# jcatalang/LUDVM

Hardware: AMD Instinct MI355X
Metric: biot_savart_pair_interactions_per_s (higher is better)
Workload: dtype f32

## Files before the change

ludvm_amd/csrc/context.hip:

```cpp
#include "ctx.hpp"

namespace ludvm_host {

int fail(ludvm_ctx* c, int code, const std::string& msg) {
  if (c) c->err = msg;
  return code;
}

int fail_hip(ludvm_ctx* c, const char* what, hipError_t e) {
  return fail(c, e == hipErrorOutOfMemory ? LUDVM_E_NOMEM : LUDVM_E_HIP,
              std::string(what) + ": " + hipGetErrorString(e));
}

int ensure(ludvm_ctx* c, Buf& b, size_t bytes) {
  if (bytes <= b.cap) return LUDVM_OK;
  HIPCHK(c, hipStreamSynchronize(c->stream));
  if (c->stream_b) HIPCHK(c, hipStreamSynchronize(c->stream_b));
  if (b.p) HIPCHK(c, hipFree(b.p));
  b.p = nullptr;
  b.cap = 0;
  size_t want = std::max(bytes, (size_t)1 << 20);
  HIPCHK(c, hipMalloc(&b.p, want));
  b.cap = want;
  return LUDVM_OK;
}

int h2d(ludvm_ctx* c, void* dst, const void* src, size_t bytes) {
  if (bytes == 0) return LUDVM_OK;
  if (bytes > kPinBytes / 4) {
    HIPCHK(c, hipMemcpyAsync(dst, src, bytes, hipMemcpyHostToDevice, c->stream));
    HIPCHK(c, hipStreamSynchronize(c->stream));
    return LUDVM_OK;
  }
  if (!c->pin) HIPCHK(c, hipHostMalloc(reinterpret_cast<void**>(&c->pin), kPinBytes, hipHostMallocDefault));
  const size_t need = (bytes + 63) & ~(size_t)63;
  if (c->pin_off + need > kPinBytes) {
    HIPCHK(c, hipStreamSynchronize(c->stream));
    c->pin_off = 0;
  }
  std::memcpy(c->pin + c->pin_off, src, bytes);
  HIPCHK(c, hipMemcpyAsync(dst, c->pin + c->pin_off, bytes, hipMemcpyHostToDevice, c->stream));
  c->pin_off += need;
  return LUDVM_OK;
}

int d2h_small_sync(ludvm_ctx* c, const void* dsrc, size_t bytes, void** host_view) {
  if (!c->pin_out) HIPCHK(c, hipHostMalloc(reinterpret_cast<void**>(&c->pin_out), kPinOutBytes, hipHostMallocDefault));
  HIPCHK(c, hipMemcpyAsync(c->pin_out, dsrc, bytes, hipMemcpyDeviceToHost, c->stream));
  HIPCHK(c, hipStreamSynchronize(c->stream));
  *host_view = c->pin_out;
  return LUDVM_OK;
}

}

extern "C" {

int ludvm_abi_version(void) { return LUDVM_ABI_VERSION; }

int ludvm_create(int device_ordinal, ludvm_ctx** out) {
  const char* small_env = LUDVM_EXP_ENV("LUDVM_SMALL_TILE_MAX");
  if (!out) return LUDVM_E_ARG;
  *out = nullptr;
  int ndev = 0;
  if (hipGetDeviceCount(&ndev) != hipSuccess || ndev <= 0) return LUDVM_E_NODEVICE;
  if (device_ordinal < 0 || device_ordinal >= ndev) return LUDVM_E_ARG;
  ludvm_ctx* c = new (std::nothrow) ludvm_ctx();
  if (!c) return LUDVM_E_NOMEM;
  c->device = device_ordinal;
  if (hipSetDevice(device_ordinal) != hipSuccess || hipGetDeviceProperties(&c->prop, device_ordinal) != hipSuccess) {
    delete c;
    return LUDVM_E_HIP;
  }
  if (std::strncmp(c->prop.gcnArchName, "gfx950", 6) != 0) {
    delete c;
    return LUDVM_E_NODEVICE;
  }
  if (hipStreamCreateWithFlags(&c->own_stream, hipStreamNonBlocking) != hipSuccess) {
    delete c;
    return LUDVM_E_HIP;
  }
  c->stream = c->own_stream;
  if (const char* gk = LUDVM_EXP_ENV("LUDVM_GRID_KERNEL")) {
    const std::string k(gk);
    c->grid_kernel = k == "row" || k == "1" ? 1 : (k == "patch2" ? 3 : (k == "patch4" ? 4 : 2));
  }
  if (const char* fp = LUDVM_EXP_ENV("LUDVM_FEW_PACKED")) c->few_packed = !(fp[0] == '0');
  if (const char* sq = LUDVM_EXP_ENV("LUDVM_SYM_QUAD")) c->sym_quad = !(sq[0] == '0');
  if (const char* sq = LUDVM_EXP_ENV("LUDVM_SYM_QUAD_MIN_TILES")) c->sym_quad_min_tiles = std::max<long long>(16, std::atoll(sq));
  if (const char* xr = LUDVM_EXP_ENV("LUDVM_XCD_RUN")) c->xcd_run = std::max(0, std::atoi(xr));
  if (const char* ti = LUDVM_EXP_ENV("LUDVM_SYM_TAIL_ITEMS")) c->sym_tail_items = std::max<long long>(0, std::atoll(ti));
  if (const char* mx = LUDVM_EXP_ENV("LUDVM_SYM_MIXED")) {
    if (mx[0] == '1') c->tune_sym_rsplit = -1;
    if (mx[0] == '0') c->tune_sym_rsplit = -2;
  }
  if (small_env) { c->small_tile_max = std::atoll(small_env); c->small_tile_max_f64 = std::min<long long>(c->small_tile_max, 12000); }
  const char* small64_env = LUDVM_EXP_ENV("LUDVM_SMALL_TILE_MAX_F64");
  if (small64_env) c->small_tile_max_f64 = std::atoll(small64_env);
  *out = c;
  return LUDVM_OK;
}

int ludvm_destroy(ludvm_ctx* c) {
  if (!c) return LUDVM_E_ARG;
  (void)hipSetDevice(c->device);
  (void)hipStreamSynchronize(c->stream);
  if (c->stream_b) (void)hipStreamSynchronize(c->stream_b);
  comm_release(c);
  for (auto& t : c->pending) { (void)hipEventDestroy(t.e0); (void)hipEventDestroy(t.e1); }
  for (auto& t : c->pool) { (void)hipEventDestroy(t.e0); (void)hipEventDestroy(t.e1); }
  void* bufs[] = {c->part.p, c->acc.p, c->symsc.p, c->arena.p, c->orderws.p, c->x64, c->z64, c->g64, c->xh, c->xl, c->zh, c->zl, c->g32,
                  c->xr, c->zr, c->cx, c->cz, c->march_tab.p, c->march_kin.p, c->march_rows.p, c->march_state.p, c->march_hist.p,
                  c->probe_xz.p, c->probe_shift.p, c->probe_part.p, c->probe_out.p, c->tracer_seed.p, c->tracer_release.p,
                  c->tracer_shift.p, c->tracer_cur.p, c->tracer_part.p, c->tracer_out.p, c->survey_xz.p, c->survey_shift.p, c->survey_sums.p,
                  c->survey_part.p, c->ens_in.p, c->ens_work.p, c->ens_out.p};
  for (void* p : bufs)
    if (p) (void)hipFree(p);
  for (auto& e : c->march_ev)
    if (e) (void)hipEventDestroy(e);
  if (c->ev_fork) (void)hipEventDestroy(c->ev_fork);
  if (c->ev_join) (void)hipEventDestroy(c->ev_join);
  if (c->stream_b) (void)hipStreamDestroy(c->stream_b);
  if (c->progress) (void)hipHostFree(c->progress);
  if (c->pin) (void)hipHostFree(c->pin);
  if (c->pin_out) (void)hipHostFree(c->pin_out);
  if (c->own_stream) (void)hipStreamDestroy(c->own_stream);
  delete c;
  return LUDVM_OK;
}

const char* ludvm_last_error(const ludvm_ctx* c) { return c ? c->err.c_str() : "null context"; }

int ludvm_device_info(ludvm_ctx* c, int* cu_count, int* clock_khz, long long* hbm_bytes, char* name, int name_len) {
  if (!c) return LUDVM_E_ARG;
  if (cu_count) *cu_count = c->prop.multiProcessorCount;
  if (clock_khz) *clock_khz = c->prop.clockRate;
  if (hbm_bytes) *hbm_bytes = (long long)c->prop.totalGlobalMem;
  if (name && name_len > 0) {
    std::snprintf(name, (size_t)name_len, "%s (%s)", c->prop.name, c->prop.gcnArchName);
  }
  return LUDVM_OK;
}

int ludvm_set_stream(ludvm_ctx* c, void* hip_stream, int external) {
  if (!c) return LUDVM_E_ARG;
  HIPCHK(c, hipSetDevice(c->device));
  hipStream_t next = external ? static_cast<hipStream_t>(hip_stream) : c->own_stream;
  if (next == c->stream) return LUDVM_OK;
  HIPCHK(c, hipStreamSynchronize(c->stream));
  c->pin_off = 0;
  c->stream = next;
  return LUDVM_OK;
}

int ludvm_synchronize(ludvm_ctx* c) {
  if (!c) return LUDVM_E_ARG;
  HIPCHK(c, hipSetDevice(c->device));
  HIPCHK(c, hipStreamSynchronize(c->stream));
  return LUDVM_OK;
}

int ludvm_set_tuning(ludvm_ctx* c, int targets_per_lane, int source_splits) {
  if (!c) return LUDVM_E_ARG;
  if (!(targets_per_lane == 0 || targets_per_lane == 1 || targets_per_lane == 2 || targets_per_lane == 4))
    return fail(c, LUDVM_E_ARG, "targets_per_lane must be 0, 1, 2 or 4");
  if (source_splits < 0 || source_splits > kMaxSplit) return fail(c, LUDVM_E_ARG, "source_splits out of range");
  c->tune_tpl = targets_per_lane;
  c->tune_split = source_splits;
  return LUDVM_OK;
}

int ludvm_set_sym_tuning(ludvm_ctx* c, int vortices_per_lane, int rotation_split) {
// ... 42 lines not shown
```

ludvm_amd/csrc/ctx.hpp:

```cpp
#pragma once
#pragma GCC visibility push(default)
#include "../../include/ludvm_hip.h"
#pragma GCC visibility pop
#include "pair_kernels.hpp"
#include "pair_sym_kernels.hpp"
#include "march_types.hpp"
#include "spatial_order.hpp"

#include <hip/hip_ext.h>
#include <rccl/rccl.h>
#include <dlfcn.h>

#include <algorithm>
#include <cmath>
#include <cstdio>
#include <cstdlib>
#include <cstring>
#include <string>
#include <utility>
#include <vector>

using namespace ludvm;

#ifdef LUDVM_EXPERIMENTS
#define LUDVM_EXP_ENV(name) std::getenv(name)
#else
#define LUDVM_EXP_ENV(name) static_cast<const char*>(nullptr)
#endif

struct Buf {
  void* p = nullptr;
  size_t cap = 0;
};

struct TimedLaunch {
  hipEvent_t e0, e1;
};

struct ludvm_ctx {
  int device = 0;
  hipStream_t own_stream = nullptr;
  hipStream_t stream = nullptr;
  hipDeviceProp_t prop;
  std::string err;

  int tune_tpl = 0;
  int tune_split = 0;
  int sym_mode = 1;
  int tune_sym_t = 0, tune_sym_rsplit = 0;
  int xcd_run = 0;
  long long sym_tail_items = kSymTailItems;
  int grid_kernel = 2;
  long long small_tile_max = 14000;
  bool sym_quad = true;
  long long sym_quad_min_tiles = kSymQuadMinTiles;
  bool few_packed = true;
  long long small_tile_max_f64 = 12000;

  Buf part;
  Buf acc;
  Buf symsc;
  Buf arena;
  Buf orderws;
  char* pin = nullptr;
  size_t pin_off = 0;
  char* pin_out = nullptr;
  std::vector<double> pack;

  size_t wake_cap = 0, wake_n = 0;
  double *x64 = nullptr, *z64 = nullptr, *g64 = nullptr;
  float *xh = nullptr, *xl = nullptr, *zh = nullptr, *zl = nullptr, *g32 = nullptr;
  float *xr = nullptr, *zr = nullptr, *cx = nullptr, *cz = nullptr;
  Mirrors mir() const { return Mirrors{xh, xl, zh, zl, xr, zr, cx, cz}; }

  Buf march_tab, march_kin, march_rows, march_state, march_hist;
  MarchSetup msetup{};
  size_t march_kin_rows = 0;
  double march_vcore = 0.0;
  bool march_ready = false;
  unsigned long long* progress = nullptr;
  unsigned long long* progress_dev = nullptr;
  hipEvent_t march_ev[2] = {nullptr, nullptr};
  hipStream_t stream_b = nullptr;
  hipEvent_t ev_fork = nullptr, ev_join = nullptr;
  Buf probe_xz, probe_shift, probe_part, probe_out;
  size_t probe_count = 0;
  size_t probe_rows = 0;
  bool probe_shifted = false;
  Buf tracer_seed, tracer_release, tracer_shift, tracer_cur, tracer_part, tracer_out;
  size_t tracer_count = 0;
  bool tracer_shifted = false;
  bool tracer_ran = false;
  std::vector<long long> tracer_record;
  std::vector<long long> tracer_rows;
  Buf survey_xz, survey_shift, survey_sums, survey_part;
  size_t survey_count = 0;
  bool survey_shifted = false;
  long long survey_first = 1, survey_stop = 0, survey_every = 1;
  long long survey_samples = 0;

  Buf ens_in, ens_work, ens_out;

  int shard_rank = 0, shard_world = 1;
  long long shard_min_n = 0;
  ludvm_allreduce_fn reduce_hook = nullptr;
  void* reduce_user = nullptr;
  void* ext_acc = nullptr;
  size_t ext_acc_bytes = 0;
  ncclComm_t comm = nullptr;
  int comm_rank = 0, comm_world = 1;
  bool comm_force = false;

  bool timing = false;
  std::vector<TimedLaunch> pending;
  std::vector<TimedLaunch> pool;
  double total_ms = 0.0;
  long long launches = 0;
};

namespace ludvm_host {

int fail(ludvm_ctx* c, int code, const std::string& msg);
int fail_hip(ludvm_ctx* c, const char* what, hipError_t e);

#define HIPCHK(c, call)                                     \
  do {                                                      \
    hipError_t e__ = (call);                                \
    if (e__ != hipSuccess) return fail_hip((c), #call, e__); \
  } while (0)

#define CHK(call)                     \
  do {                                \
    int rc__ = (call);                \
    if (rc__ != LUDVM_OK) return rc__; \
  } while (0)

int ensure(ludvm_ctx* c, Buf& b, size_t bytes);
constexpr size_t kPinBytes = (size_t)1 << 20;
// ... 108 lines not shown
```

ludvm_amd/csrc/launch.hip:

```cpp
#include "ctx.hpp"
#include "sym_prepare_kernels.hpp"

namespace ludvm_host {

Plan make_plan(const ludvm_ctx* c, long long nt_launch, long long ns, int precision, bool small_ok, long long plan_nt, bool grid_patch) {
  Plan p{};
  const long long nt = plan_nt > 0 ? plan_nt : nt_launch;
  const bool f64 = precision == LUDVM_PREC_F64;
  p.tile = f64 ? ((nt <= kFewTargets || ns <= c->small_tile_max_f64) ? kTileF64Few : kTileF64) : kTileF32;
  if (!f64 && small_ok && ns <= c->small_tile_max) p.tile = kTileF32Small;
  if (f64) {
    p.tpl = 1;
  } else if (c->tune_tpl == 1 || c->tune_tpl == 2 || c->tune_tpl == 4) {
    p.tpl = c->tune_tpl;
  } else {
    p.tpl = nt >= 131072 ? 2 : 1;
  }
  if (p.tile == kTileF32Small && (p.tpl != 1 || nt > 65536)) p.tile = kTileF32;
  const long long per_wg = grid_patch ? (long long)kBlock * 4 * (nt >= (1LL << 20) ? 4 : 2) : (long long)kBlock * p.tpl;
  const long long ttiles = std::max<long long>(1, (nt + per_wg - 1) / per_wg);
  const long long max_split = std::max<long long>(1, (ns + p.tile - 1) / p.tile);
  long long nsplit = c->tune_split > 0 ? c->tune_split : (kTargetBlocks + ttiles - 1) / ttiles;
  nsplit = std::max<long long>(1, std::min<long long>(std::min<long long>(nsplit, max_split), kMaxSplit));
  long long chunk = (std::max<long long>(ns, 1) + nsplit - 1) / nsplit;
// ... 101 lines not shown
        else hipLaunchKernelGGL((pair_f32<4, kTileF32, false, 1, true>), grid, dim3(kBlock), 0, c->stream, a);
      }
    } else if (p.tile == kTileF32Small) {
      hipLaunchKernelGGL((pair_f32<1, kTileF32Small, false, 0, true>), grid, dim3(kBlock), 0, c->stream, a);
    } else {
      switch (p.tpl) {
        case 1: hipLaunchKernelGGL((pair_f32<1, kTileF32, false, 0, true>), grid, dim3(kBlock), 0, c->stream, a); break;
        case 2: hipLaunchKernelGGL((pair_f32<2, kTileF32, false, 0, true>), grid, dim3(kBlock), 0, c->stream, a); break;
        default: hipLaunchKernelGGL((pair_f32<4, kTileF32, false, 0, true>), grid, dim3(kBlock), 0, c->stream, a); break;
      }
    }
  } else if (p.tile == kTileF32Small && !(a.grid_nz > 0)) {
    if (precision == LUDVM_PREC_F32X2)
      hipLaunchKernelGGL((pair_f32<1, kTileF32Small, true>), grid, dim3(kBlock), 0, c->stream, a);
    else
      hipLaunchKernelGGL((pair_f32<1, kTileF32Small, false>), grid, dim3(kBlock), 0, c->stream, a);
  } else if (precision == LUDVM_PREC_F32X2) {
    switch (p.tpl) {
      case 1: hipLaunchKernelGGL((pair_f32<1, kTileF32, true>), grid, dim3(kBlock), 0, c->stream, a); break;
      case 2: hipLaunchKernelGGL((pair_f32<2, kTileF32, true>), grid, dim3(kBlock), 0, c->stream, a); break;
      default: hipLaunchKernelGGL((pair_f32<4, kTileF32, true>), grid, dim3(kBlock), 0, c->stream, a); break;
    }
  } else if (a.grid_nz > 0 && a.grid_nz % 4 == 0 && c->tune_tpl == 0) {
    const int prows = grid_patch_rows(c, a, p);
    grid = dim3((unsigned)grid_kernel_blocks(a, prows), grid.y, 1);
    if (prows == 4) {
      hipLaunchKernelGGL((pair_f32<16, kTileF32, false, 2>), grid, dim3(kBlock), 0, c->stream, a);
    } else if (prows == 2) {
      if (p.tile == kTileF32Small) hipLaunchKernelGGL((pair_f32<8, kTileF32Small, false, 2>), grid, dim3(kBlock), 0, c->stream, a);
      else hipLaunchKernelGGL((pair_f32<8, kTileF32, false, 2>), grid, dim3(kBlock), 0, c->stream, a);
    } else {
      if (p.tile == kTileF32Small) hipLaunchKernelGGL((pair_f32<4, kTileF32Small, false, 1>), grid, dim3(kBlock), 0, c->stream, a);
      else hipLaunchKernelGGL((pair_f32<4, kTileF32, false, 1>), grid, dim3(kBlock), 0, c->stream, a);
    }
  } else {
    switch (p.tpl) {
      case 1: hipLaunchKernelGGL((pair_f32<1, kTileF32, false>), grid, dim3(kBlock), 0, c->stream, a); break;
      case 2: hipLaunchKernelGGL((pair_f32<2, kTileF32, false>), grid, dim3(kBlock), 0, c->stream, a); break;
      default: hipLaunchKernelGGL((pair_f32<4, kTileF32, false>), grid, dim3(kBlock), 0, c->stream, a); break;
    }
  }
  HIPCHK(c, hipGetLastError());
  CHK(timed_end(c, t, active));
  return LUDVM_OK;
}

int induce_device(ludvm_ctx* c, const PairArgs& a, long long nt, long long ns, int precision, void* u, void* w,
                  long long plan_nt) {
  if (nt == 0) return LUDVM_OK;
  const size_t elt = precision == LUDVM_PREC_F64 ? sizeof(double) : sizeof(float);
  if (ns == 0) {
    HIPCHK(c, hipMemsetAsync(u, 0, (size_t)nt * elt, c->stream));
    HIPCHK(c, hipMemsetAsync(w, 0, (size_t)nt * elt, c->stream));
    return LUDVM_OK;
  }
  const bool grid_generic = a.grid_nz > 0 && !(a.grid_nz % 4 == 0 && c->tune_tpl == 0);
  const bool grid_patch = a.grid_nz > 0 && !grid_generic && precision == LUDVM_PREC_F32;
  Plan p = make_plan(c, nt, ns, precision, !grid_generic, plan_nt, grid_patch);
  CHK(launch_pair(c, a, p, precision, u, w));
  if (p.nsplit > 1) {
    if (precision == LUDVM_PREC_F64)
      hipLaunchKernelGGL(finish_sum<double>, dim3(blocks_for(nt)), dim3(kBlock), 0, c->stream,
                         static_cast<const double*>(c->part.p), nt, p.nt_pad, p.nsplit, static_cast<double*>(u),
                         static_cast<double*>(w));
    else
      hipLaunchKernelGGL(finish_sum<float>, dim3(blocks_for(nt)), dim3(kBlock), 0, c->stream,
                         static_cast<const float*>(c->part.p), nt, p.nt_pad, p.nsplit, static_cast<float*>(u),
                         static_cast<float*>(w));
    HIPCHK(c, hipGetLastError());
  }
  return LUDVM_OK;
}

static_assert(64 * 8 == LUDVM_SYM_TILE, "the multi-GPU entry points always use the 512-vortex tile");

SymKnobs sym_knobs(const ludvm_ctx* c) {
  SymKnobs k;
  k.sym_mode = c->sym_mode;
  k.tile_t = c->tune_sym_t;
  k.tune_split = c->tune_split;
  k.tune_rsplit = c->tune_sym_rsplit;
  k.quad = c->sym_quad;
  k.quad_min_tiles = c->sym_quad_min_tiles;
  k.tail_items = c->sym_tail_items;
  return k;
}
long long sym_threshold(const ludvm_ctx* c, bool march) { return sym_min_n(sym_knobs(c), march); }
bool use_symmetric(const ludvm_ctx* c, long long n, double vc4, bool march) {
  return sym_use(sym_knobs(c), n, (float)vc4 > 0.0f, march);
}
int sym_tile_t(const ludvm_ctx* c, long long n, bool hilo) { return sym_tile(sym_knobs(c), n, hilo); }

int launch_sym_tiles(ludvm_ctx* c, int T, const SymOperands& o, long long n, long long i_first, long long i_count, double vc4,
                     const long long* n_dev, long long n_lo, bool sharded) {
  if (n >= (1LL << 31)) return fail(c, LUDVM_E_ARG, "the symmetric kernel indexes vortices with 32 bits: n < 2^31");
  SymArgs a{};
  a.x = o.x; a.z = o.z; a.g = o.g; a.n = n;
  a.n_dev = n_dev;
  a.xl = o.xl; a.zl = o.zl;
  a.cx = o.cx; a.cz = o.cz;
  const SymKnobs k = sym_knobs(c);
  const SymVariant v = sym_variant(k, n, T, o.xl && o.zl);
  const SymGeom& gm = v.g;
  a.tune_split = k.tune_split;
  a.tune_rsplit = v.tune_rsplit;
  a.shard_rank = (n_dev && sharded) ? c->shard_rank : 0;
  a.shard_world = (n_dev && sharded) ? c->shard_world : 1;
  a.tail_items = k.tail_items;
  a.ntiles = gm.ntiles;
  a.dmax = gm.dmax;
  a.i_first = i_first;
  a.i_count = i_count;
  a.ysplit = gm.ysplit;
  a.rsplit = gm.rsplit;
  a.ytail = gm.ytail;
  a.rbulk = gm.rbulk;
  a.xcd_run = c->xcd_run;
  a.acc_u = o.acc_u;
  a.acc_w = o.acc_w;
  a.scale = o.scale;
  a.bad = o.bad;
  a.vc4 = (float)vc4;
  long long blocks = sym_blocks(i_count, gm.ysplit, gm.rsplit, gm.ytail, gm.rbulk, c->xcd_run);
  if (n_dev) blocks = std::max(blocks, sym_grid_bound(k, v, false, n_lo, n, c->xcd_run));
  if (!n_dev && i_count == 0) return LUDVM_OK;
  blocks = std::max<long long>(blocks, 1);
  if (v.quad) {
    if (i_first % 4 != 0 || (i_count % 4 != 0 && i_first + i_count != gm.ntiles))
      return fail(c, LUDVM_E_ARG, "symmetric kernel, quad variant: an owner's tile block must start and end on multiples of 4 tiles");
    TimedLaunch tq{};
    bool act = false;
    CHK(timed_begin(c, tq, act));
    SymArgs d = a;
    d.diag_only = 1;
    const long long dblocks = std::max<long long>(1, sym_blocks(n_dev ? gm.ntiles : i_count, 1, 1, 0, 1, c->xcd_run));
    hipLaunchKernelGGL((pair_sym_f32<8, false, 1>), dim3((unsigned)dblocks), dim3(kBlock), 0, c->stream, d);
    long long qblocks = quad_blocks(n_dev ? gm.ntiles : i_count, v.q.ysplit, c->xcd_run);
    if (n_dev) qblocks = std::max(qblocks, sym_grid_bound(k, v, true, n_lo, n, c->xcd_run));
    hipLaunchKernelGGL((pair_sym_quad_f32<8>), dim3((unsigned)std::max<long long>(qblocks, 1)), dim3(kBlock), 0, c->stream, a);
    HIPCHK(c, hipGetLastError());
    CHK(timed_end(c, tq, act));
    return LUDVM_OK;
  }
  TimedLaunch t{};
  bool active = false;
  CHK(timed_begin(c, t, active));
  const dim3 grid((unsigned)blocks);
  const dim3 blk(kBlock);
#define LUDVM_SYM_LAUNCH(TT, HH)                                                                              \
  switch (gm.rsplit) {                                                                                        \
    case 0: hipLaunchKernelGGL((pair_sym_f32<TT, HH, 0>), grid, blk, 0, c->stream, a); break;                 \
    case 1: hipLaunchKernelGGL((pair_sym_f32<TT, HH, 1>), grid, blk, 0, c->stream, a); break;                 \
    case 2: hipLaunchKernelGGL((pair_sym_f32<TT, HH, 2>), grid, blk, 0, c->stream, a); break;                 \
    default: hipLaunchKernelGGL((pair_sym_f32<TT, HH, 4>), grid, blk, 0, c->stream, a); break;                \
  }
  if (v.hilo) { LUDVM_SYM_LAUNCH(4, true) }
  else if (v.T == 8) { LUDVM_SYM_LAUNCH(8, false) }
  else { LUDVM_SYM_LAUNCH(4, false) }
#undef LUDVM_SYM_LAUNCH
  HIPCHK(c, hipGetLastError());
  CHK(timed_end(c, t, active));
  return LUDVM_OK;
}

int acc_buffer(ludvm_ctx* c, long long nt_pad, long long** acc) {
  const size_t bytes = ((size_t)2 * (size_t)nt_pad + 2) * sizeof(long long);
  if (c->ext_acc) {
    if (bytes > c->ext_acc_bytes) return fail(c, LUDVM_E_NOMEM, "the accumulator buffer given to ludvm_set_shard is too small");
    *acc = static_cast<long long*>(c->ext_acc) + 2;
    return LUDVM_OK;
  }
  CHK(ensure(c, c->acc, bytes));
  *acc = static_cast<long long*>(c->acc.p) + 2;
  return LUDVM_OK;
}

bool sharded_at(const ludvm_ctx* c, long long n) { return (c->shard_world > 1 || c->comm_force) && n >= c->shard_min_n; }

void shard_tiles(const ludvm_ctx* c, long long ntiles, long long* first, long long* count) {
  unsigned long long f, cnt;
  shard_block((unsigned long long)ntiles, c->shard_rank, c->shard_world, &f, &cnt);
  *first = (long long)f;
  *count = (long long)cnt;
}

int launch_sym_prepare(ludvm_ctx* c, const float* g, long long n, double vc4, SymScale* scale, long long* bad) {
  const long long nparts = (n + kPrepChunk - 1) / kPrepChunk;
  if (nparts <= 1) {
    hipLaunchKernelGGL(sym_prepare, dim3(1), dim3(kPrepBlock), 0, c->stream, g, n, vc4, scale, bad, (double*)nullptr);
  } else {
    CHK(ensure(c, c->symsc, 128 + (size_t)nparts * sizeof(double)));
    double* partial = reinterpret_cast<double*>(static_cast<char*>(c->symsc.p) + 128);
    hipLaunchKernelGGL(sym_prepare, dim3((unsigned)nparts), dim3(kPrepBlock), 0, c->stream, g, n, vc4, scale, bad, partial);
    hipLaunchKernelGGL(sym_prepare_final, dim3(1), dim3(64), 0, c->stream, partial, (int)nparts, vc4, scale, bad);
  }
  HIPCHK(c, hipGetLastError());
  return LUDVM_OK;
}

int launch_sym(ludvm_ctx* c, SymOperands o, long long n, double vc4, long long* nt_pad_out, const long long** acc_out,
               const long long** bad_out, const long long* n_dev, long long n_lo) {
  const long long nt_pad = (n + 63) / 64 * 64;
  long long* acc = nullptr;
  CHK(acc_buffer(c, nt_pad, &acc));
  CHK(ensure(c, c->symsc, 128 + (size_t)((n + kPrepChunk - 1) / kPrepChunk) * sizeof(double)));
  HIPCHK(c, hipMemsetAsync(acc - 2, 0, ((size_t)2 * (size_t)nt_pad + 2) * sizeof(long long), c->stream));
  o.acc_u = acc;
  o.acc_w = acc + nt_pad;
  if (!o.scale) {
    CHK(launch_sym_prepare(c, o.g, n, vc4, ctx_scale(c), ctx_bad(c)));
    o.scale = ctx_scale(c);
    o.bad = ctx_bad(c);
  }
  const bool sharded = sharded_at(c, n);
  if (sharded) o.bad = acc - 2;
  const int T = sym_tile_t(c, n, o.xl && o.zl);
  const long long ntiles = (n + 64LL * T - 1) / (64LL * T);
  long long first = 0, count = ntiles;
  if (sharded) shard_tiles(c, ntiles, &first, &count);
  CHK(launch_sym_tiles(c, T, o, n, first, count, vc4, n_dev, n_lo, sharded));
  if (sharded) CHK(reduce_accumulators(c, acc, nt_pad));
  *nt_pad_out = nt_pad;
// ... 50 lines not shown
```

ludvm_amd/csrc/pair_sym_kernels.hpp:

```cpp
#pragma once
#include <hip/hip_runtime.h>
#include "pair_kernels.hpp"
#include "sym_rule.hpp"

namespace ludvm {

struct SymScale {
  float scale;
  float pad;
  double inv;
};

struct SymArgs {
  const float* x; const float* z; const float* g;
  const float* xl; const float* zl;
  const float* cx; const float* cz;
  long long n;
  long long ntiles;
  long long dmax;
  long long i_first;
  long long i_count;
  int ysplit;
  int rsplit;
  int ytail;
// ... 520 lines not shown
      const int d = D - w;
      const unsigned Iw = I0 + (unsigned)w;
      const bool own = Iw < i_first + i_count && Iw < ntiles;
      return own && ((d >= 1 && d <= (int)dmax) || (even && d == dtot && Iw < ntiles / 2));
    };
    const bool valid = valid_of(wv);
    const bool any = valid_of(0) || valid_of(1) || valid_of(2) || valid_of(3);
    if (any) store_quarter();
    Org oj[NS];
#pragma unroll
    for (int q = 0; q < NS; ++q) oj[q] = to_scalars(poj[q]);
    __syncthreads();
    if (dd + 1 < per) fetch_quarter(dd + 1);
    if (!any) continue;
    f32x2 bu[H], bw[H];
#pragma unroll
    for (int m = 0; m < H; ++m) { bu[m] = (f32x2){0.f, 0.f}; bw[m] = (f32x2){0.f, 0.f}; }
    if (valid) {
#pragma unroll
      for (int q = 0; q < NS; ++q) {
        if (local) refer_targets(oj[q]);
        for (int k = 0; k < 64; k += 2) {
          const int pos0 = ((k & 32) ? lane32x4 : lane * 4) + (k & 31) * 4;
#pragma unroll
          for (int rr = 0; rr < 2; ++rr) {
            const int pos = pos0 + 4 * rr;
            f32x2 xj[2], zj[2], gj[2];
            load_plane(lx, q, pos, xj); load_plane(lz, q, pos, zj); load_plane(lg, q, pos, gj);
#pragma unroll
            for (int mm = 0; mm < 2; ++mm) {
              const int m = 2 * q + mm;
#pragma unroll
              for (int t = 0; t < T; ++t) {
                const f32x2 dx = pk_sub_sel(xq[rr][t / 2], xj[mm], t & 1);
                const f32x2 dz = pk_sub_sel(zq[rr][t / 2], zj[mm], t & 1);
                f32x2 r2 = dx * dx;
                r2 = __builtin_elementwise_fma(dz, dz, r2);
                const f32x2 qq = __builtin_elementwise_fma(r2, r2, vc4);
                const f32x2 sv = {__builtin_amdgcn_rsqf(qq.x), __builtin_amdgcn_rsqf(qq.y)};
                const f32x2 sj = sv * gj[mm];
                const f32x2 si = pk_mul_sel(sv, gp[t / 2], t & 1, sj);
                au[t] = __builtin_elementwise_fma(dz, sj, au[t]);
                aw[t] = __builtin_elementwise_fma(dx, sj, aw[t]);
                bu[m] = __builtin_elementwise_fma(dz, si, bu[m]);
                bw[m] = __builtin_elementwise_fma(dx, si, bw[m]);
              }
            }
#pragma unroll
            for (int mm = 0; mm < 2; ++mm) { bu[2 * q + mm] = dpp_rol1(bu[2 * q + mm]); bw[2 * q + mm] = dpp_rol1(bw[2 * q + mm]); }
          }
        }
      }
    }
#pragma unroll
    for (int m = 0; m < H; ++m) {
      ex[wv][(4 * m + 0) * 64 + lane] = bu[m].x; ex[wv][(4 * m + 1) * 64 + lane] = bu[m].y;
      ex[wv][(4 * m + 2) * 64 + lane] = bw[m].x; ex[wv][(4 * m + 3) * 64 + lane] = bw[m].y;
    }
    __syncthreads();
#pragma unroll 1
    for (int c = wv; c < 2 * T; c += kWaves) {
      float v = 0.0f;
#pragma unroll
      for (int w = 0; w < kWaves; ++w) v += ex[w][c * 64 + lane];
      const unsigned j = J * W + lane + 64u * (2 * (c / 4) + (c & 1));
      if (j < n) fx_add((c & 2) ? &a.acc_w[j] : &a.acc_u[j], -v, fxs);
    }
  }

  if (mine) {
#pragma unroll
    for (int t = 0; t < T; ++t) {
      const unsigned i = I * W + lane + 64u * t;
      if (i < n) {
        const float su = au[t].x + au[t].y, sw = aw[t].x + aw[t].y;
        fx_add(&a.acc_u[i], su, fxs); fx_add(&a.acc_w[i], sw, fxs);
        chk += su + sw;
      }
    }
  }
  if (!(__builtin_fabsf(chk) < __builtin_inff())) atomicAdd(reinterpret_cast<unsigned long long*>(a.bad), 1ULL);
}

constexpr int kPrepBlock = 1024;
__device__ __forceinline__ void sym_scale_from_sum(double sum_abs, double vc4, SymScale* out, long long* bad) {
  const double vc = sqrt(sqrt(vc4));
  const double bound = sum_abs / (1.4142135623730951 * vc);
  int e = 0;
  if (bound > 0.0 && bound < 1.0e300) (void)frexp(bound, &e);
  else if (!(bound == 0.0) && bad) atomicAdd(reinterpret_cast<unsigned long long*>(bad), 1ULL);
  int k = 61 - e;
  if (k > 120) k = 120;
  if (k < -120) k = -120;
  out->scale = (float)ldexp(1.0, k);
  out->pad = 0.0f;
  out->inv = ldexp(1.0, -k);
}

__device__ __forceinline__ double block_abs_sum(const float* g, long long first, long long count) {
  __shared__ double part[kPrepBlock / 64];
  double s[8] = {0, 0, 0, 0, 0, 0, 0, 0};
  const long long end = first + count;
  long long i = first + threadIdx.x;
  for (; i + 7 * kPrepBlock < end; i += 8 * kPrepBlock) {
#pragma unroll
    for (int k = 0; k < 8; ++k) s[k] += (double)__builtin_fabsf(g[i + k * kPrepBlock]);
  }
  for (int k = 0; i < end; i += kPrepBlock, ++k) s[k & 7] += (double)__builtin_fabsf(g[i]);
  double t = ((s[0] + s[1]) + (s[2] + s[3])) + ((s[4] + s[5]) + (s[6] + s[7]));
#pragma unroll
  for (int off = 32; off > 0; off >>= 1) t += __shfl_down(t, off, 64);
  __syncthreads();
  if ((threadIdx.x & 63) == 0) part[threadIdx.x >> 6] = t;
  __syncthreads();
  double tot = 0.0;
  for (int w = 0; w < (int)(blockDim.x >> 6); ++w) tot += part[w];
  return tot;
}

constexpr long long kPrepChunk = 65536;

__device__ __forceinline__ float fx_read(const long long* acc, long long i, const SymScale* sc, bool bad) {
  if (bad) return __builtin_nanf("");
  return (float)((double)acc[i] * sc->inv);
}
__device__ __forceinline__ float fx_read(const long long* acc, long long i, const SymScale* sc, const long long* bad) {
  return fx_read(acc, i, sc, *bad != 0);
}

constexpr int kFoilChunk = 256;
__device__ __forceinline__ void staged_sources_on(bool on, double xi, double zi, const double* x64, const double* z64,
                                                  const float* g32, long long first, int nsrc, float vc4, float& fu,
                                                  float& fw, int nextra = 0, const double* extra = nullptr) {
  __shared__ float fx[kFoilChunk], fz[kFoilChunk], fg[kFoilChunk];
  fu = 0.0f; fw = 0.0f;
  const int ntot = nsrc + nextra;
  if (ntot <= 0) return;
  const double ax = nsrc > 0 ? x64[first] : extra[0], az = nsrc > 0 ? z64[first] : extra[2];
  const float xr = (float)(xi - ax), zr = (float)(zi - az);
  for (int base = 0; base < ntot; base += kFoilChunk) {
    const int cnt = ntot - base < kFoilChunk ? ntot - base : kFoilChunk;
    __syncthreads();
    for (int t = threadIdx.x; t < cnt; t += blockDim.x) {
      const int q = base + t;
      if (q < nsrc) {
        fx[t] = (float)(x64[first + q] - ax);
        fz[t] = (float)(z64[first + q] - az);
        fg[t] = g32[first + q];
      } else {
        fx[t] = (float)(extra[q - nsrc] - ax);
        fz[t] = (float)(extra[2 + q - nsrc] - az);
        fg[t] = (float)extra[4 + q - nsrc];
      }
    }
    __syncthreads();
    if (on) {
      for (int j = 0; j < cnt; ++j) {
        const float dx = xr - fx[j], dz = zr - fz[j];
        const float r2 = __builtin_fmaf(dz, dz, dx * dx);
        const float k = fg[j] * __builtin_amdgcn_rsqf(__builtin_fmaf(r2, r2, vc4));
        fu = __builtin_fmaf(dz, k, fu);
        fw = __builtin_fmaf(dx, k, fw);
      }
    }
  }
}
// ... 3 lines not shown
```

ludvm_amd/csrc/sym_rule.hpp:

```cpp
#pragma once
#include <cstddef>
#include <cstdio>
#ifndef __HIPCC__
#define __host__
#define __device__
#endif

namespace ludvm {

constexpr long long kSymTargetWaves = 8 * 65536;
constexpr long long kSymMaxSplit = 64;
constexpr long long kSymMaxSplitTuned = 1024;
constexpr long long kXcds = 8;
constexpr long long kSymMaxRsplit = 4;
constexpr long long kSymMinItems = 10500;
constexpr long long kSymTailItems = 1536;
struct SymGeom { long long ntiles, dmax, dtot; int ysplit, rsplit, ytail, rbulk; };
struct XcdShare { unsigned lo, n; };
__host__ __device__ inline XcdShare xcd_share(unsigned units, unsigned e) {
  const unsigned lo = (unsigned)((unsigned long long)units * e / (unsigned)kXcds);
  return XcdShare{lo, (unsigned)((unsigned long long)units * (e + 1) / (unsigned)kXcds) - lo};
}
__host__ __device__ inline unsigned xcd_run(unsigned ys, int k) {
  return k > 0 ? (unsigned)k : (ys > 0 ? (ys + (unsigned)kXcds - 1) / (unsigned)kXcds : 1);
// ... 95 lines not shown
    rbulk = (int)rb;
  } else {
    while (rs < (I)kSymMaxRsplit && nt1 * ys * rs < (I)kSymMinItems) rs *= 2;
    if (tune_rsplit != -2 && rs < (I)kSymMaxRsplit) {
      rbulk = (int)rs;
      rs = 0;
      const I yt = (tail_items + nt1 - 1) / nt1;
      ytail = (int)(yt > ys ? ys : yt);
    }
  }
  ysplit = (int)ys;
  rsplit = (int)rs;
}
__host__ __device__ inline SymGeom sym_geometry(long long n, int T, int tune_split, int tune_rsplit,
                                                 long long tail_items = kSymTailItems) {
  SymGeom g;
  sym_geometry_t<long long>(n, T, tune_split, tune_rsplit, tail_items, g.ntiles, g.dmax, g.dtot, g.ysplit, g.rsplit, g.ytail,
                            g.rbulk);
  return g;
}

constexpr unsigned kQuad = 4;
constexpr unsigned kQuadSplit = 128;
struct QuadGeom { unsigned ntiles, dmax, dtot, Dtot; int ysplit, per, nlong, pshort; };
template <typename I>
__host__ __device__ inline QuadGeom quad_geometry(I n, int T, int tune_split) {
  QuadGeom g;
  const I W = (I)(64 * T);
  const I nt = (n + W - 1) / W;
  g.ntiles = (unsigned)nt;
  g.dmax = nt > 0 ? (unsigned)((nt - 1) / 2) : 0;
  g.dtot = g.dmax + ((nt % 2 == 0 && nt > 1) ? 1u : 0u);
  g.Dtot = g.dtot + (kQuad - 1);
  if (tune_split > 0) {
    unsigned ys = (unsigned)tune_split;
    if (ys > (unsigned)kSymMaxSplitTuned) ys = (unsigned)kSymMaxSplitTuned;
    if (ys > g.Dtot) ys = g.Dtot;
    if (ys < 1) ys = 1;
    g.per = (int)((g.Dtot + ys - 1) / ys);
    g.ysplit = (int)((g.Dtot + (unsigned)g.per - 1) / (unsigned)g.per);
    g.nlong = g.ysplit;
    g.pshort = g.per;
    return g;
  }
  const unsigned u = (g.Dtot + kQuadSplit - 1) / kQuadSplit;
  const unsigned P = 2 * (u > 0 ? u : 1), ps = u / 4 > 0 ? u / 4 : 1;
  const unsigned nlong = (g.Dtot - g.Dtot / 8) / P;
  const unsigned rest = g.Dtot - nlong * P;
  g.per = (int)P;
  g.pshort = (int)ps;
  g.nlong = (int)nlong;
  g.ysplit = (int)(nlong + (rest + ps - 1) / ps);
  if (g.ysplit < 1) g.ysplit = 1;
  return g;
}
__host__ __device__ inline void quad_chunk(const QuadGeom& g, unsigned yq, int& lo, int& hi) {
  const bool lg = (int)yq < g.nlong;
  lo = 1 + (lg ? (int)yq * g.per : g.nlong * g.per + ((int)yq - g.nlong) * g.pshort);
  hi = lo + (lg ? g.per : g.pshort);
  if (hi > (int)g.Dtot + 1) hi = (int)g.Dtot + 1;
}
__host__ __device__ inline long long quad_blocks(long long i_count, int ysplit, int k = 0) {
  const unsigned quads = (unsigned)((i_count + kQuad - 1) / kQuad);
  long long most = 0;
  for (unsigned x = 0; x < (unsigned)kXcds; ++x) {
    const long long wg = (long long)xcd_items(quads, (unsigned)ysplit, x, 0, (unsigned)ysplit, k);
    most = wg > most ? wg : most;
  }
  return kXcds * most;
}

constexpr long long kSymMinN = 16384;
constexpr long long kSymT8MinN = 36864;
constexpr long long kSymMinNMarch = 11264;
constexpr long long kSymQuadMinTiles = 640;

struct SymKnobs {
  int sym_mode = 1;
  int tile_t = 0;
  int tune_split = 0;
  int tune_rsplit = 0;
  bool quad = true;
  long long quad_min_tiles = kSymQuadMinTiles;
  long long tail_items = kSymTailItems;
  long long t8_min_n = kSymT8MinN;
};

inline long long sym_min_n(const SymKnobs& k, bool march) {
  return k.sym_mode == 1 ? (march ? kSymMinNMarch : kSymMinN) : (long long)k.sym_mode;
}
inline bool sym_use(const SymKnobs& k, long long n, bool core, bool march) {
  return k.sym_mode != 0 && core && n >= sym_min_n(k, march);
}
inline int sym_tile(const SymKnobs& k, long long n, bool hilo) {
  if (hilo) return 4;
  if (k.tile_t == 4 || k.tile_t == 8) return k.tile_t;
  return n >= k.t8_min_n ? 8 : 4;
}

struct SymVariant {
  int T;
  bool hilo;
  int tune_rsplit;
  SymGeom g;
  bool quad;
  QuadGeom q;
};
inline SymVariant sym_variant(const SymKnobs& k, long long n, int T, bool hilo) {
  SymVariant v{};
  v.T = hilo ? 4 : T;
  v.hilo = hilo;
  v.tune_rsplit = (hilo && k.tune_rsplit == 0) ? -2 : k.tune_rsplit;
  v.g = sym_geometry(n, v.T, k.tune_split, v.tune_rsplit, k.tail_items);
  const bool one_wave_items = v.g.rsplit == 1 || (v.g.rsplit == 0 && v.g.rbulk == 1);
  v.quad = v.T == 8 && !hilo && v.g.ntiles >= 16 &&
           (k.tune_rsplit == -4 || (k.quad && one_wave_items && k.tune_rsplit == 0 && v.g.ntiles >= k.quad_min_tiles));
  if (v.quad) v.q = quad_geometry<long long>(n, 8, k.tune_split);
  return v;
}
inline void sym_kernel_name(const SymVariant& v, char* out, size_t len) {
  if (v.quad) std::snprintf(out, len, "pair_sym_quad_f32<8>");
  else std::snprintf(out, len, "pair_sym_f32<%d, %s, %d, %s>", v.T, v.hilo ? "true" : "false", v.g.rsplit,
                     v.g.rsplit != 1 ? "true" : "false");
}

inline long long sym_grid_bound(const SymKnobs& k, const SymVariant& v, bool quad_kernel, long long n_lo, long long n, int xcd_run) {
  const long long W = 64LL * v.T;
  long long most = 0;
  for (long long nt = ((n_lo > 1 ? n_lo : 1) + W - 1) / W; nt <= (n + W - 1) / W; ++nt) {
    const SymGeom q = sym_geometry(nt * W, v.T, k.tune_split, v.g.rsplit == 0 ? -1 : v.g.rsplit, k.tail_items);
    const long long b = quad_kernel ? quad_blocks(nt, quad_geometry<long long>(nt * W, v.T, k.tune_split).ysplit, xcd_run)
                                    : sym_blocks(q.ntiles, q.ysplit, v.g.rsplit, q.ytail, q.rbulk, xcd_run);
    most = b > most ? b : most;
  }
  return most;
}

}
```

Baseline: 9003 billion.

## Add quad16 symmetric pair kernel with doubled per-lane target tile

```diff
diff --git a/ludvm_amd/csrc/context.hip b/ludvm_amd/csrc/context.hip
--- a/ludvm_amd/csrc/context.hip
+++ b/ludvm_amd/csrc/context.hip
@@ -88,6 +88,7 @@
   if (const char* fp = LUDVM_EXP_ENV("LUDVM_FEW_PACKED")) c->few_packed = !(fp[0] == '0');
   if (const char* sq = LUDVM_EXP_ENV("LUDVM_SYM_QUAD")) c->sym_quad = !(sq[0] == '0');
   if (const char* sq = LUDVM_EXP_ENV("LUDVM_SYM_QUAD_MIN_TILES")) c->sym_quad_min_tiles = std::max<long long>(16, std::atoll(sq));
+  if (const char* sq = LUDVM_EXP_ENV("LUDVM_SYM_QUAD16")) c->sym_quad16 = !(sq[0] == '0');
   if (const char* xr = LUDVM_EXP_ENV("LUDVM_XCD_RUN")) c->xcd_run = std::max(0, std::atoi(xr));
   if (const char* ti = LUDVM_EXP_ENV("LUDVM_SYM_TAIL_ITEMS")) c->sym_tail_items = std::max<long long>(0, std::atoll(ti));
   if (const char* mx = LUDVM_EXP_ENV("LUDVM_SYM_MIXED")) {
diff --git a/ludvm_amd/csrc/ctx.hpp b/ludvm_amd/csrc/ctx.hpp
--- a/ludvm_amd/csrc/ctx.hpp
+++ b/ludvm_amd/csrc/ctx.hpp
@@ -54,6 +54,7 @@
   long long small_tile_max = 14000;
   bool sym_quad = true;
   long long sym_quad_min_tiles = kSymQuadMinTiles;
+  bool sym_quad16 = true;
   bool few_packed = true;
   long long small_tile_max_f64 = 12000;
 
diff --git a/ludvm_amd/csrc/launch.hip b/ludvm_amd/csrc/launch.hip
--- a/ludvm_amd/csrc/launch.hip
+++ b/ludvm_amd/csrc/launch.hip
@@ -207,6 +207,7 @@
   k.tune_rsplit = c->tune_sym_rsplit;
   k.quad = c->sym_quad;
   k.quad_min_tiles = c->sym_quad_min_tiles;
+  k.quad16 = c->sym_quad16;
   k.tail_items = c->sym_tail_items;
   return k;
 }
@@ -262,7 +263,9 @@
     hipLaunchKernelGGL((pair_sym_f32<8, false, 1>), dim3((unsigned)dblocks), dim3(kBlock), 0, c->stream, d);
     long long qblocks = quad_blocks(n_dev ? gm.ntiles : i_count, v.q.ysplit, c->xcd_run);
     if (n_dev) qblocks = std::max(qblocks, sym_grid_bound(k, v, true, n_lo, n, c->xcd_run));
-    hipLaunchKernelGGL((pair_sym_quad_f32<8>), dim3((unsigned)std::max<long long>(qblocks, 1)), dim3(kBlock), 0, c->stream, a);
+    const dim3 qgrid((unsigned)std::max<long long>(qblocks, 1));
+    if (sym_quad16(k, v, a.cx == nullptr)) hipLaunchKernelGGL((pair_sym_quad16_f32<8>), qgrid, dim3(kBlock), 0, c->stream, a);
+    else hipLaunchKernelGGL((pair_sym_quad_f32<8>), qgrid, dim3(kBlock), 0, c->stream, a);
     HIPCHK(c, hipGetLastError());
     CHK(timed_end(c, tq, act));
     return LUDVM_OK;
diff --git a/ludvm_amd/csrc/pair_sym_kernels.hpp b/ludvm_amd/csrc/pair_sym_kernels.hpp
--- a/ludvm_amd/csrc/pair_sym_kernels.hpp
+++ b/ludvm_amd/csrc/pair_sym_kernels.hpp
@@ -626,6 +626,209 @@
   if (!(__builtin_fabsf(chk) < __builtin_inff())) atomicAdd(reinterpret_cast<unsigned long long*>(a.bad), 1ULL);
 }
 
+template <int T>
+__global__ void __launch_bounds__(kBlock) __attribute__((amdgpu_waves_per_eu(2)))
+pair_sym_quad16_f32(SymArgs a) {
+  static_assert(T == 8, "the quad variant is built for the 512-vortex tile");
+  constexpr int H = T / 2, NS = T / 4;
+  constexpr int TI = 2 * T, HI = TI / 2;
+  constexpr unsigned W = 64u * T;
+  constexpr int kWaves = kBlock / 64;
+  static_assert(kWaves == (int)kQuad, "one I tile per wave");
+  __shared__ __attribute__((aligned(16))) float slab[3][(T / 4) * kPlane];
+  __shared__ __attribute__((aligned(16))) float ex[kWaves][2 * T * 64];
+  static_assert(2 * T * 64 == TI * 64, "a wave's ex row also carries half of its own-side sums between its halves");
+
+  unsigned n = (unsigned)a.n, i_first = (unsigned)a.i_first, i_count = (unsigned)a.i_count;
+  if (a.n_dev) {
+    n = (unsigned)*a.n_dev;
+    const unsigned nt = (n + W - 1) / W;
+    i_first = 0;
+    i_count = nt;
+    if (a.shard_world > 1) {
+      unsigned long long f, cnt;
+      shard_block(nt, a.shard_rank, a.shard_world, &f, &cnt);
+      i_first = (unsigned)f;
+      i_count = (unsigned)cnt;
+    }
+  }
+  const QuadGeom gm = quad_geometry<unsigned>(n, T, a.tune_split);
+  const unsigned ntiles = gm.ntiles, dmax = gm.dmax;
+  const int dtot = (int)gm.dtot;
+  const bool even = (ntiles % 2 == 0) && ntiles > 1;
+
+  const int lane = threadIdx.x & 63;
+  const int wv = __builtin_amdgcn_readfirstlane((int)(threadIdx.x >> 6));
+  const unsigned xcd = blockIdx.x % (unsigned)kXcds, qb = blockIdx.x / (unsigned)kXcds;
+  const unsigned quads = (i_count + kQuad - 1) / kQuad;
+  unsigned yq, quad;
+  if (!xcd_item(quads, (unsigned)gm.ysplit, xcd, 0, (unsigned)gm.ysplit, qb, yq, quad, a.xcd_run)) return;
+  const unsigned I0 = i_first + kQuad * quad;
+  const unsigned I = I0 + (unsigned)wv;
+  const bool mine = I < i_first + i_count && I < ntiles;
+  int D_lo, D_hi;
+  quad_chunk(gm, yq, D_lo, D_hi);
+  const int per = D_hi - D_lo;
+
+  float* const lx = slab[0];
+  float* const lz = slab[1];
+  float* const lg = slab[2];
+
+  const unsigned p32 = (unsigned)(lane & 31);
+  const bool upper = (lane & 32) != 0;
+  f32x2 xt[HI], zt[HI], gp[HI], au[TI], aw[TI];
+  {
+    float x0[TI], z0[TI], g0[TI];
+#pragma unroll
+    for (int t = 0; t < TI; ++t) {
+      const unsigned i = I * W + p32 + 32u * t;
+      const unsigned nl = mine ? n : 0u;
+      x0[t] = load_or(a.x, i, nl, kPadPosF); z0[t] = load_or(a.z, i, nl, kPadPosF); g0[t] = load_or(a.g, i, nl, 0.0f);
+      au[t] = (f32x2){0.f, 0.f}; aw[t] = (f32x2){0.f, 0.f};
+    }
+#pragma unroll
+    for (int h = 0; h < HI; ++h) {
+      gp[h] = (f32x2){g0[2 * h], g0[2 * h + 1]};
+      xt[h] = (f32x2){x0[2 * h], x0[2 * h + 1]};
+      zt[h] = (f32x2){z0[2 * h], z0[2 * h + 1]};
+    }
+  }
+  const f32x2 vc4 = {a.vc4, a.vc4};
+  const float fxs = a.scale->scale;
+  auto load_plane = [&](const float* l, int q, int pos4, f32x2 (&out)[2]) {
+    const f32x4 V = *reinterpret_cast<const f32x4*>(&l[q * kPlane + pos4]);
+    out[0] = (f32x2){V.x, V.y};
+    out[1] = (f32x2){V.z, V.w};
+  };
+  float chk = 0.0f;
+
+  const int qhome = 32 * (wv & 1) + (lane >> 1);
+  float pjx[2], pjz[2], pjg[2];
+  auto partner_of = [&](int dd) -> unsigned {
+    unsigned J = I0 + (unsigned)(D_lo + dd);
+    if (J >= ntiles) J -= ntiles;
+    return J;
+  };
+  auto fetch_quarter = [&](int dd) {
+    const unsigned J = (D_lo + dd < D_hi) ? partner_of(dd) : I0;
+    const unsigned Jc = J < ntiles ? J : 0u;
+#pragma unroll
+    for (int s = 0; s < 2; ++s) {
+      const unsigned j = Jc * W + (unsigned)qhome + 64u * (unsigned)(4 * (wv >> 1) + 2 * (lane & 1) + s);
+      pjx[s] = load_or(a.x, j, n, kPadPosF); pjz[s] = load_or(a.z, j, n, kPadPosF); pjg[s] = load_or(a.g, j, n, 0.0f);
+    }
+  };
+  auto store_quarter = [&]() {
+    const int at = (wv >> 1) * kPlane + 128 * (wv & 1) + 2 * lane;
+    auto put = [&](float* l, const float (&v)[2]) {
+      *reinterpret_cast<f32x2*>(&l[at]) = (f32x2){v[0], v[1]};
+      if ((wv & 1) == 0) *reinterpret_cast<f32x2*>(&l[at + 256]) = (f32x2){v[0], v[1]};
+    };
+    put(lx, pjx); put(lz, pjz); put(lg, pjg);
+  };
+
+  fetch_quarter(0);
+  for (int dd = 0; dd < per; ++dd) {
+    const int D = D_lo + dd;
+    if (D >= D_hi) break;
+    const unsigned J = partner_of(dd);
+    auto valid_of = [&](int w) -> bool {
+      const int d = D - w;
+      const unsigned Iw = I0 + (unsigned)w;
+      const bool own = Iw < i_first + i_count && Iw < ntiles;
+      return own && ((d >= 1 && d <= (int)dmax) || (even && d == dtot && Iw < ntiles / 2));
+    };
+    const bool valid = valid_of(wv);
+    const bool any = valid_of(0) || valid_of(1) || valid_of(2) || valid_of(3);
+    if (any) store_quarter();
+    __syncthreads();
+    if (dd + 1 < per) fetch_quarter(dd + 1);
+    if (!any) continue;
+    f32x2 bu[H], bw[H];
+#pragma unroll
+    for (int m = 0; m < H; ++m) { bu[m] = (f32x2){0.f, 0.f}; bw[m] = (f32x2){0.f, 0.f}; }
+    if (valid) {
+#pragma unroll
+      for (int q = 0; q < NS; ++q) {
+        for (int k = 0; k < 32; k += 2) {
+          const int pos0 = (lane + k) * 4;
+#pragma unroll
+          for (int rr = 0; rr < 2; ++rr) {
+            const int pos = pos0 + 4 * rr;
+            f32x2 xj[2], zj[2], gj[2];
+            load_plane(lx, q, pos, xj); load_plane(lz, q, pos, zj); load_plane(lg, q, pos, gj);
+#pragma unroll
+            for (int mm = 0; mm < 2; ++mm) {
+              const int m = 2 * q + mm;
+#pragma unroll
+              for (int t = 0; t < TI; ++t) {
+                const f32x2 dx = pk_sub_sel(xt[t / 2], xj[mm], t & 1);
+                const f32x2 dz = pk_sub_sel(zt[t / 2], zj[mm], t & 1);
+                f32x2 r2 = dx * dx;
+                r2 = __builtin_elementwise_fma(dz, dz, r2);
+                const f32x2 qq = __builtin_elementwise_fma(r2, r2, vc4);
+                const f32x2 sv = {__builtin_amdgcn_rsqf(qq.x), __builtin_amdgcn_rsqf(qq.y)};
+                const f32x2 sj = sv * gj[mm];
+                const f32x2 si = pk_mul_sel(sv, gp[t / 2], t & 1, sj);
+                au[t] = __builtin_elementwise_fma(dz, sj, au[t]);
+                aw[t] = __builtin_elementwise_fma(dx, sj, aw[t]);
+                bu[m] = __builtin_elementwise_fma(dz, si, bu[m]);
+                bw[m] = __builtin_elementwise_fma(dx, si, bw[m]);
+              }
+            }
+#pragma unroll
+            for (int mm = 0; mm < 2; ++mm) { bu[2 * q + mm] = dpp_rol1(bu[2 * q + mm]); bw[2 * q + mm] = dpp_rol1(bw[2 * q + mm]); }
+          }
+#pragma unroll
+          for (int t = 0; t < TI; ++t) { asm("" : "+v"(au[t])); asm("" : "+v"(aw[t])); }
+        }
+      }
+    }
+    const int home = (lane + 32) & 63;
+#pragma unroll
+    for (int m = 0; m < H; ++m) {
+      ex[wv][(4 * m + 0) * 64 + home] = bu[m].x; ex[wv][(4 * m + 1) * 64 + home] = bu[m].y;
+      ex[wv][(4 * m + 2) * 64 + home] = bw[m].x; ex[wv][(4 * m + 3) * 64 + home] = bw[m].y;
+    }
+    __syncthreads();
+#pragma unroll 1
+    for (int c = wv; c < 2 * T; c += kWaves) {
+      float v = 0.0f;
+#pragma unroll
+      for (int w = 0; w < kWaves; ++w) v += ex[w][c * 64 + lane];
+      const unsigned j = J * W + lane + 64u * (2 * (c / 4) + (c & 1));
+      if (j < n) fx_add((c & 2) ? &a.acc_w[j] : &a.acc_u[j], -v, fxs);
+    }
+  }
+
+  __syncthreads();
+  auto pick = [](bool c, f32x2 y, f32x2 n_) -> f32x2 { return (f32x2){c ? y.x : n_.x, c ? y.y : n_.y}; };
+  if (mine) {
+#pragma unroll
+    for (int s = 0; s < T; ++s) {
+      const f32x2 us = pick(upper, au[s], au[s + T]), ws = pick(upper, aw[s], aw[s + T]);
+      ex[wv][(2 * s) * 64 + lane] = us.x + us.y;
+      ex[wv][(2 * s + 1) * 64 + lane] = ws.x + ws.y;
+    }
+    __builtin_amdgcn_fence(__ATOMIC_RELEASE, "wavefront");
+    __builtin_amdgcn_wave_barrier();
+    __builtin_amdgcn_fence(__ATOMIC_ACQUIRE, "wavefront");
+#pragma unroll
+    for (int s = 0; s < T; ++s) {
+      const f32x2 uk = pick(upper, au[s + T], au[s]), wk = pick(upper, aw[s + T], aw[s]);
+      const float mu = uk.x + uk.y, mw = wk.x + wk.y;
+      const float ou = ex[wv][(2 * s) * 64 + (lane ^ 32)], ow = ex[wv][(2 * s + 1) * 64 + (lane ^ 32)];
+      const unsigned i = I * W + p32 + 32u * (unsigned)(s + (upper ? T : 0));
+      if (i < n) {
+        const float su = upper ? ou + mu : mu + ou, sw = upper ? ow + mw : mw + ow;
+        fx_add(&a.acc_u[i], su, fxs); fx_add(&a.acc_w[i], sw, fxs);
+        chk += su + sw;
+      }
+    }
+  }
+  if (!(__builtin_fabsf(chk) < __builtin_inff())) atomicAdd(reinterpret_cast<unsigned long long*>(a.bad), 1ULL);
+}
+
 constexpr int kPrepBlock = 1024;
 __device__ __forceinline__ void sym_scale_from_sum(double sum_abs, double vc4, SymScale* out, long long* bad) {
   const double vc = sqrt(sqrt(vc4));
diff --git a/ludvm_amd/csrc/sym_rule.hpp b/ludvm_amd/csrc/sym_rule.hpp
--- a/ludvm_amd/csrc/sym_rule.hpp
+++ b/ludvm_amd/csrc/sym_rule.hpp
@@ -201,6 +201,7 @@
   int tune_rsplit = 0;
   bool quad = true;
   long long quad_min_tiles = kSymQuadMinTiles;
+  bool quad16 = true;
   long long tail_items = kSymTailItems;
   long long t8_min_n = kSymT8MinN;
 };
@@ -237,8 +238,9 @@
   if (v.quad) v.q = quad_geometry<long long>(n, 8, k.tune_split);
   return v;
 }
-inline void sym_kernel_name(const SymVariant& v, char* out, size_t len) {
-  if (v.quad) std::snprintf(out, len, "pair_sym_quad_f32<8>");
+inline bool sym_quad16(const SymKnobs& k, const SymVariant& v, bool plain) { return v.quad && plain && k.quad16; }
+inline void sym_kernel_name(const SymVariant& v, char* out, size_t len, bool quad16 = false) {
+  if (v.quad) std::snprintf(out, len, quad16 ? "pair_sym_quad16_f32<8>" : "pair_sym_quad_f32<8>");
   else std::snprintf(out, len, "pair_sym_f32<%d, %s, %d, %s>", v.T, v.hilo ? "true" : "false", v.g.rsplit,
                      v.g.rsplit != 1 ? "true" : "false");
 }
```

Result: no change. 9072 billion (median of 6 runs) (+0.8%).
